# aweisberg/cassandra-accord

Measured on AMD Instinct MI355X. Metric: txn-key conflict pairs resolved/sec (node), higher is better.
Workload: dtype u32/u64 (integer); 1 GPU; config2: KeyDeps batch, 1M txns x 8 keys, zipf(0.99) over 1M keys, p_write 0.5, uncommitted window 10k, per-GPU CommandStore snapshot; key_distribution=zipf, keys_permuted=True, n_txn_per_gpu=1000000, pairs_per_gpu=8000000, dep_edges_per_gpu=35349420, parallelism=keyspace shards x1 (independent CommandStores)

## Files before the change

### cassandra-accord_amd/accord_amd/_lib.py

```python
from __future__ import annotations

import ctypes as C
import os

HERE = os.path.dirname(os.path.abspath(__file__))
LIB_PATH = os.environ.get("ACC_LIB_PATH") or os.path.join(HERE, "libaccord_amd.so")

ACC_OK, ACC_E_ARG, ACC_E_STATE, ACC_E_NOMEM, ACC_E_DEVICE, ACC_E_CAP = 0, -1, -2, -3, -4, -5
ACC_MEM_HOST, ACC_MEM_DEVICE = 0, 1
ACC_OPT_TIMING = 1
ACC_OPT_FORCE_REPLAY = 2
ACC_OPT_NO_WINDOW_TIER = 4
ACC_OPT_TIER_GRID_SHIFT = 16
ACC_OPT_RD_WIDE_SORT = 8
ACC_OPT_PD_SERIAL = 16
ACC_LV_AUTO, ACC_LV_LDS_WALK, ACC_LV_WINDOWED, ACC_LV_WAVES = 0, 1, 2, 3
ACC_STARTED_BEFORE, ACC_STARTED_AFTER, ACC_STARTED_ANY = 0, 1, 2
ACC_DEP_WITH, ACC_DEP_WITHOUT, ACC_DEP_ANY = 0, 1, 2
ACC_STATUS_ANY, ACC_STATUS_IS_PROPOSED, ACC_STATUS_IS_STABLE = 0, 1, 2
ACC_FULL_EXECUTES_AFTER = 1
ACC_LATEST_PROPOSAL, ACC_LATEST_COMMIT = 0, 1
RECOVERY_SCANS = {
    "acceptedOrCommittedStartedBeforeWithoutWitnessing": (ACC_STARTED_BEFORE, ACC_DEP_WITHOUT, ACC_STATUS_IS_PROPOSED, True),
    "stableStartedBeforeAndWitnessed": (ACC_STARTED_BEFORE, ACC_DEP_WITH, ACC_STATUS_IS_STABLE, False),
    "hasAcceptedOrCommittedStartedAfterWithoutWitnessing": (ACC_STARTED_AFTER, ACC_DEP_WITHOUT, ACC_STATUS_IS_PROPOSED, False),
    "hasStableExecutesAfterWithoutWitnessing": (ACC_STARTED_ANY, ACC_DEP_WITHOUT, ACC_STATUS_IS_STABLE, False),
}

u64p = C.POINTER(C.c_uint64)
u32p = C.POINTER(C.c_uint32)
# ... 553 lines not shown
```

### cassandra-accord_amd/accord_amd/deps.py

```python
from __future__ import annotations

import ctypes as C
from dataclasses import dataclass

import numpy as np

from . import _lib as L


class AccordError(RuntimeError):
    code = None


class IllegalArgumentException(AccordError):
    code = L.ACC_E_ARG


class IllegalStateException(AccordError):
    code = L.ACC_E_STATE


class DeviceError(AccordError):
    code = L.ACC_E_DEVICE

# ... 4 lines not shown

_ERRORS = {L.ACC_E_ARG: IllegalArgumentException, L.ACC_E_STATE: IllegalStateException,
           L.ACC_E_DEVICE: DeviceError, L.ACC_E_NOMEM: DeviceError, L.ACC_E_CAP: CapacityError}


def _ptr(a: np.ndarray):
    return C.c_void_p(a.ctypes.data)


class Context:

    LV_TIERS = {"auto": 0, "lds": 1, "windowed": 2, "waves": 3}

    def __init__(self, device: int = 0, timing: bool = False, force_replay: bool = False, *, cfk_hot: int = 0,
                 lv_tier: str = "auto", lv_chunk: int = 0, no_window_tier: bool = False, rd_wide_sort: bool = False,
                 pd_serial: bool = False, cfq_wave_cap: int = 0, wave_grid_max: int = 0, tier_grid_max: int = 0):
        self.timing_enabled = timing
        self.device = device
        self._lib = L.load()
        h = C.c_void_p()
        flags = ((L.ACC_OPT_TIMING if timing else 0) | (L.ACC_OPT_FORCE_REPLAY if force_replay else 0) |
                 (L.ACC_OPT_NO_WINDOW_TIER if no_window_tier else 0) | (L.ACC_OPT_RD_WIDE_SORT if rd_wide_sort else 0) |
                 (L.ACC_OPT_PD_SERIAL if pd_serial else 0))
        if not 0 <= int(tier_grid_max) <= 0xFFFF:
            raise ValueError("tier_grid_max must be within 0..65535")
        flags |= int(tier_grid_max) << L.ACC_OPT_TIER_GRID_SHIFT
        opts = L.Opts(flags, int(wave_grid_max), int(cfk_hot), self.LV_TIERS[lv_tier], int(lv_chunk), int(cfq_wave_cap))
        rc = self._lib.acc_create(device, C.byref(opts), C.byref(h))
        if rc != L.ACC_OK:
            raise _ERRORS.get(rc, AccordError)(f"acc_create failed ({rc})")
        self._h = h
        self._keep = []

    def close(self):
        if getattr(self, "_h", None):
            self._lib.acc_destroy(self._h)
            self._h = None

# ... 1176 lines not shown
```

### cassandra-accord_amd/csrc/api.hip

```cpp
#include "dict.hpp"
#include <exception>
#include <thread>

namespace acc {
void keydeps_batch(acc_ctx *ctx, const acc_batch_in *in, acc_keydeps_view *view);
void keydeps_mixed(acc_ctx *ctx, const acc_range_batch_in *in, acc_keydeps_view *view, SharedDict *shared = nullptr);
void keydeps_merge(acc_ctx *ctx, const acc_merge_in *in, acc_merge_view *view);
void levelise(acc_ctx *ctx, const acc_graph_in *in, uint32_t *level, uint32_t *order, uint32_t *n_levels);
void rangedeps_batch(acc_ctx *ctx, const acc_range_batch_in *in, acc_rangedeps_view *view, const SharedDict *shared = nullptr);
void shard_pack(acc_ctx *ctx, const acc_batch_in *in, acc_frag_streams *out, bool ctx_alloc);
void shard_merge(acc_ctx *ctx, const acc_frag_recv *in, acc_merge_view *view);
void deps_merge(acc_ctx *ctx, const acc_deps_merge_in *in, acc_deps_merge_view *view);
void rmm_invert(acc_ctx *ctx, const acc_rmm_batch *in, acc_csr_view *out);
void rmm_slice(acc_ctx *ctx, const acc_rmm_batch *in, const acc_ranges_in *select, acc_slice_view *out);
void rangedeps_stab(acc_ctx *ctx, const acc_rmm_batch *rd, const acc_stab_in *q, acc_stab_view *out);
void rmm_without(acc_ctx *ctx, const acc_rmm_batch *in, const acc_ts_cols *txn, const acc_txn_sets *set_a,
                 const acc_txn_sets *set_b, acc_without_view *out);
void recovery_deps_reduce(acc_ctx *ctx, const acc_deps_merge_in *cw, const acc_deps_merge_in *anw, acc_recovery_deps_view *view);
void map_reduce_full(acc_ctx *ctx, const acc_batch_in *in, const acc_recovery_in *q, acc_keydeps_view *view);
void map_reduce_full_ranges(acc_ctx *ctx, const acc_range_cmds_in *c, const acc_recovery_ranges_in *q, acc_rangedeps_view *view);
void latest_deps_merge(acc_ctx *ctx, const acc_latest_in *in, acc_latest_view *view);
void deps_from_json(acc_ctx *ctx, const acc_json_in *in, acc_json_deps_view *view);
void deps_to_json(acc_ctx *ctx, const acc_json_out_in *in, acc_json_out *out);
void cfk_update(acc_ctx *ctx, acc_cfk *cfk, const acc_batch_in *in);
// ... 70 lines not shown
{
    if (!ctx) return;
    (void)hipSetDevice(ctx->device);
    if (ctx->stream) (void)hipStreamSynchronize(ctx->stream);
    for (auto &kv : ctx->bufs)
        if (kv.second.ptr) (void)hipFree(kv.second.ptr);
    for (void *p : ctx->graveyard) (void)hipFree(p);
    for (auto &p : ctx->pending) { (void)hipEventDestroy(p.start); (void)hipEventDestroy(p.stop); }
    for (auto e : ctx->event_pool) (void)hipEventDestroy(e);
    for (int i = 0; i < acc_ctx::NAUX; ++i) {
        if (ctx->aux[i]) { (void)hipStreamSynchronize(ctx->aux[i]); (void)hipStreamDestroy(ctx->aux[i]); }
        if (ctx->join_ev[i]) (void)hipEventDestroy(ctx->join_ev[i]);
    }
    if (ctx->fork_ev) (void)hipEventDestroy(ctx->fork_ev);
    if (ctx->lane_ev) (void)hipEventDestroy(ctx->lane_ev);
    if (ctx->pinned) (void)hipHostFree(ctx->pinned);
    if (ctx->stream) (void)hipStreamDestroy(ctx->stream);
    acc_ctx *child = ctx->child;
    delete ctx;
    ctx_destroy(child);
}

}

extern "C" {

const char *acc_last_error(const acc_ctx *ctx) { return ctx ? ctx->last_error.c_str() : "null context"; }

int acc_sync(acc_ctx *ctx)
{
// ... 617 lines not shown
```

### cassandra-accord_amd/csrc/ctx.hpp

```cpp
#pragma once

#include <hip/hip_runtime.h>

#include <algorithm>
#include <cstdint>
#include <cstdio>
#include <cstring>
#include <string>
#include <unordered_map>
#include <vector>

#include "../../include/accord_amd.h"

namespace acc {

struct Error {
    int code;
    std::string msg;
};

[[noreturn]] inline void fail(int code, const std::string &msg) { throw Error{code, msg}; }

constexpr int BLOCK = 256;
constexpr int WAVES = BLOCK / 64;
// ... 20 lines not shown

struct PendingEvent {
    int slot;
    hipEvent_t start, stop;
};

}

struct acc_ctx {
    int device = 0;
    hipStream_t stream = nullptr;
    static constexpr int NAUX = 3;
    hipStream_t aux[NAUX] = {};
    hipEvent_t fork_ev = nullptr, join_ev[NAUX] = {};
    hipEvent_t lane_ev = nullptr;
    bool lane_open = false;
    hipStream_t launch_stream = nullptr;
    struct ScanState {
        size_t cap = 0, dirty[2] = {0, 0};
        int par = 0;
    };
    ScanState scan_st[2];
    int scan_lane() const { return !launch_stream ? 0 : launch_stream == aux[0] ? 1 : -1; }
    struct OsState {
        size_t cap = 0, dirty[2] = {0, 0};
        int par = 0;
    };
    std::unordered_map<std::string, OsState> os_state;
    uint32_t flags = 0;
    acc_opts opts{};
// ... 62 lines not shown
        return static_cast<T *>(b.ptr);
    }

    void swap_buf(const char *name, void *&ptr, size_t &bytes)
    {
        acc::Buf &b = bufs[ns.empty() ? std::string(name) : ns + name];
        std::swap(b.ptr, ptr);
        std::swap(b.bytes, bytes);
    }

    const void *buf_ptr(const char *name) const
    {
        auto it = bufs.find(ns.empty() ? std::string(name) : ns + name);
        return it == bufs.end() ? nullptr : it->second.ptr;
    }

    hipEvent_t take_event()
    {
        if (!event_pool.empty()) {
            hipEvent_t e = event_pool.back();
            event_pool.pop_back();
            return e;
        }
        hipEvent_t e;
        ACC_HIP(hipEventCreate(&e));
        return e;
    }

    int slot(const char *name)
    {
// ... 8 lines not shown
    void resolve_timing()
    {
        for (auto &p : pending) {
            float ms = 0;
            ACC_HIP(hipEventElapsedTime(&ms, p.start, p.stop));
            slots[p.slot].total_ms += ms;
            slots[p.slot].launches += 1;
            event_pool.push_back(p.start);
            event_pool.push_back(p.stop);
        }
        pending.clear();
    }

    hipStream_t cur() const { return launch_stream ? launch_stream : stream; }

    void fork(int k)
    {
        if (!fork_ev) {
            ACC_HIP(hipEventCreateWithFlags(&fork_ev, hipEventDisableTiming));
            ACC_HIP(hipEventCreateWithFlags(&lane_ev, hipEventDisableTiming));
            for (int i = 0; i < NAUX; ++i) {
                ACC_HIP(hipStreamCreateWithFlags(&aux[i], hipStreamNonBlocking));
                ACC_HIP(hipEventCreateWithFlags(&join_ev[i], hipEventDisableTiming));
            }
        }
        ACC_HIP(hipEventRecord(fork_ev, stream));
        for (int i = 0; i < k; ++i) ACC_HIP(hipStreamWaitEvent(aux[i], fork_ev, 0));
    }
    void join(int k)
    {
        for (int i = 0; i < k; ++i) {
            ACC_HIP(hipEventRecord(join_ev[i], aux[i]));
            ACC_HIP(hipStreamWaitEvent(stream, join_ev[i], 0));
        }
        launch_stream = nullptr;
    }

    void lane_fork() { fork(1); lane_open = true; }
    void lane_join() { if (lane_open) { join(1); lane_open = false; } }
    void lane_mark() { ACC_HIP(hipEventRecord(lane_ev, aux[0])); }
    void lane_wait() { ACC_HIP(hipStreamWaitEvent(stream, lane_ev, 0)); }

// ... 112 lines not shown
```

### cassandra-accord_amd/csrc/keydeps.hip

```cpp
#include "keydeps.hpp"

#include <vector>

namespace acc {


struct TxnInfoArgs {
    uint32_t n = 0;
    const uint8_t *status = nullptr;
    const uint64_t *tl = nullptr;
    uint4 *tinfo = nullptr;
    uint32_t *bigflag = nullptr;
};

__device__ __forceinline__ void txn_info_one(uint32_t t, uint32_t n, const uint32_t *rank, const uint8_t *status,
                                             const uint64_t *tl, const uint32_t *key_off, uint4 *tinfo, uint32_t *bigflag)
{
    if (bigflag) bigflag[t] = 0;
    const uint32_t kind = (uint32_t)(tl[t] >> 1) & 7u;
    tinfo[t] = make_uint4(rank[t], rank[n + t], (uint32_t)status[t] | (kind << 3), key_off[t]);
}

__global__ __launch_bounds__(BLOCK) void k_pair_keys(size_t P, const uint64_t *__restrict__ key_code,
                                                     const uint32_t *__restrict__ owner, const uint32_t *__restrict__ key_off,
// ... 1836 lines not shown




constexpr int ST_G = 16;
constexpr int ST_N2 = 128;
constexpr int ST_SLOT = ST_N2;
constexpr uint32_t ST_RAW = 1024;
constexpr int MK_G = 8;

__global__ __launch_bounds__(BLOCK) void k_v3_mark(uint32_t n, const uint32_t *__restrict__ key_off,
                                                   const uint32_t *__restrict__ irec32, const uint4 *__restrict__ rec,
                                                   uint32_t *__restrict__ psz, uint32_t raw_cap,
                                                   uint32_t *__restrict__ bigflag, uint64_t *__restrict__ szA,
                                                   uint64_t *__restrict__ szK, uint64_t *__restrict__ any16,
                                                   uint64_t *__restrict__ eb, uint32_t *__restrict__ runflag)
{
    const uint32_t t = (blockIdx.x * BLOCK + threadIdx.x) / MK_G, sub = threadIdx.x & (MK_G - 1);
    if (t >= n) return;
    const uint32_t j0 = key_off[t], nk = key_off[t + 1] - j0;
    const bool run_rec = bigflag[t] != 0;
    const bool maybe_big = run_rec || nk > 8u;
    uint32_t e = 0, kd = 0, raw = 0;
    for (uint32_t c0 = 0; c0 < nk; c0 += MK_G) {
        if (c0 + sub < nk) {
            const uint32_t w = irec32[IREC_W * (size_t)(j0 + c0 + sub) + 7];
            const uint32_t ej = w & ~REC_INLINE_FLAG;
            e += ej;
            kd += ej != 0;
            if (run_rec && !(w & REC_INLINE_FLAG)) {
                const uint4 *r = rec + 4 * (size_t)(j0 + c0 + sub);
                const uint4 r1 = r[1], r2 = r[2], r3 = r[3];
                raw += r1.z + r1.w + r2.x + r2.y + r2.z + r2.w + r3.y;
            }
            if (maybe_big) psz[j0 + c0 + sub] = ej;
        }
    }
#pragma unroll
    for (int d = 1; d < MK_G; d <<= 1) {
        e += __shfl_xor(e, d, 64);
        kd += __shfl_xor(kd, d, 64);
        raw += __shfl_xor(raw, d, 64);
    }
    const bool big = nk > (uint32_t)ST_G || e > (uint32_t)ST_N2 || (run_rec && raw > raw_cap);
    if (sub == 0) {
        bigflag[t] = big ? 1u : 0u;
        runflag[t] = run_rec && !big ? 1u : 0u;
        szA[t] = (uint64_t)kd + e;
        szK[t] = kd;
        eb[t] = big ? e : 0u;
        if (big && e && nk > 8 && nk <= 16 && !*any16) atomicOr((unsigned long long *)any16, 1ull);
    }
}


__global__ __launch_bounds__(BLOCK) void k_v3_compact(uint32_t n, const uint32_t *__restrict__ bigflag,
                                                      const uint32_t *__restrict__ bpos, uint32_t *__restrict__ blist)
{
    const uint32_t t = blockIdx.x * BLOCK + threadIdx.x;
    if (t < n && bigflag[t]) blist[bpos[t]] = t;
}
__global__ __launch_bounds__(BLOCK) void k_v3_route(uint32_t nbig, const uint32_t *__restrict__ blist,
                                                    const uint32_t *__restrict__ key_off, const uint64_t *__restrict__ eb,
                                                    int big_ok, int win_ok, uint32_t *__restrict__ med_list,
                                                    uint32_t *__restrict__ big_list, uint32_t *__restrict__ fb_list,
                                                    uint32_t *__restrict__ w8_list, uint32_t *__restrict__ w16_list,
                                                    uint64_t *__restrict__ gstat)
{
    const uint32_t i = blockIdx.x * BLOCK + threadIdx.x;
    bool med = false, bg = false, fb = false, w8 = false, w16 = false;
    uint32_t t = 0;
    uint64_t E = 0;
    if (i < nbig) {
        t = blist[i];
        E = eb[t];
// ... 76 lines not shown
            b.u_cnt[t] = 0;
        }
    }
}

struct V3Stream {
    V2View v;
    const uint32_t *key_off, *bigflag, *txn_of_rank;
    const uint32_t *list;
    const uint4 *rec, *irec;
    const uint64_t *arena_off, *kd_off;
    uint64_t *u_cnt_out;
    int32_t *arena;
    uint32_t *key_idx, *dep_scr;
    uint64_t *err;
    uint32_t n, ntiles;
};

template <int G>
__device__ __forceinline__ uint32_t group_inclusive(uint32_t x, uint32_t sub)
{
#pragma unroll
    for (uint32_t d = 1; d < (uint32_t)G; d <<= 1) {
        const uint32_t u = __shfl_up(x, d, 64);
        if (sub >= d) x += u;
    }
    return x;
}

template <class T>
// ... 35 lines not shown
            }
        }
    }
#pragma unroll
    for (int r = 0; r < R; ++r) buf[r * G + sub] = v[r];
}

#ifdef ACC_PHASE_PROF
__device__ unsigned long long *g_st_prof;
__device__ unsigned long long *g_sr_prof;
#define ST_PH(i) ph[i] = clock64()
#else
#define ST_PH(i) ((void)0)
#endif

#ifndef ACC_ST_WAVES
#define ACC_ST_WAVES 24
#endif
template <class EntT, int NT, int G, int N2, bool LIST, bool RUNS>
__global__ __launch_bounds__(NT, ACC_ST_WAVES * 64 / NT) void k_v3_stream(V3Stream s)
{
    constexpr int TT = NT / G;
    constexpr uint32_t KB = G <= 8 ? 3 : 4;
    static_assert(G <= 16, "entries keep the key index in 4 bits");
#ifdef ACC_PHASE_PROF
    uint64_t ph[8];
#endif
    ST_PH(0);
    __shared__ EntT ent[TT][N2];
    __shared__ uint32_t kc[TT][G];
    __shared__ uint32_t kbase[TT][G];
    __shared__ uint16_t stA[TT][G + N2];
    const uint32_t tid = threadIdx.x, lane = lane_id(), sub = lane & (G - 1), grp = tid / G, g0 = lane & (64 - G);
    const uint64_t gmask = ((1ull << G) - 1) << g0;
    const uint64_t lt = lane == 0 ? 0ull : (~0ull >> (64 - lane));
    const uint32_t tile = blockIdx.x * (NT / 64) + (tid >> 6);
    const uint32_t slot = tile * (64 / G) + lane / G;
    const bool valid = slot < s.n;
    const uint32_t t = LIST ? (valid ? s.list[slot] : 0u) : slot;
    TxnCtx c{};
    bool big = false;
    uint64_t aoff = 0, koff = 0;
    if (valid) {
        c.t = t;
        c.j0 = s.key_off[t]; c.j1 = s.key_off[t + 1];
        const uint32_t bf = s.bigflag[t];
        const uint4 ti = s.v.tinfo[t];
        aoff = s.arena_off[t]; koff = s.kd_off[t];
        c.nk = c.j1 - c.j0;
        big = bf != 0;
        c.trank = ti.x;
        c.bq = ti.y != c.trank;
        c.wk = witnesses(ti.z >> 3);
    }
// ... 440 lines not shown
    cb.tm = stage_in(ctx, "in_tm", in->txn_id.msb, n, in->mem);
    cb.tl = stage_in(ctx, "in_tl", in->txn_id.lsb, n, in->mem);
    cb.tn = stage_in(ctx, "in_tn", in->txn_id.node, n, in->mem);
    cb.em = stage_in(ctx, "in_em", in->execute_at.msb, n, in->mem);
    cb.el = stage_in(ctx, "in_el", in->execute_at.lsb, n, in->mem);
    cb.en = stage_in(ctx, "in_en", in->execute_at.node, n, in->mem);
    cb.status = stage_in(ctx, "in_status", in->status, n, in->mem);
    cb.key_code = stage_in(ctx, "in_key_code", in->key_code, P, in->mem);

    cb.g = ctx->get<uint64_t>("g", PREP_G_WORDS);
    cb.owner = ctx->get<uint32_t>("owner", P);
    prep_batch(ctx, n, P, cb.tm, cb.tl, cb.tn, cb.em, cb.el, cb.en, cb.status, cb.key_off, cb.key_code, cb.owner, cb.g, cb.dict);
    const bool overlap = pair_plan(cb) && cb.dict.fast_ok && cb.pp.rk.bits + cb.dict.rbits + 1 <= 64;
    ctx->stat("keydeps.build_overlap", overlap ? 1 : 0);
    ctx->stat("keydeps.bc_sort_passes", 0);
    if (overlap) ctx->lane_fork();
    else build_dictionary(ctx, n, cb.tm, cb.tl, cb.tn, cb.em, cb.el, cb.en, cb.g, cb.dict, true);

    cb.tinfo = ctx->get<uint4>("tinfo", n);
    cb.bigflag = ctx->get<uint32_t>("v3_bigflag", n);
    const PairSort ps = sort_pairs(ctx, cb, overlap);
    if (overlap) {
        ctx->launch_stream = ctx->aux[0];
        build_dictionary(ctx, n, cb.tm, cb.tl, cb.tn, cb.em, cb.el, cb.en, cb.g, cb.dict, true);
        ctx->lane_mark();
        bc_from_txns(ctx, cb);
        ctx->launch_stream = nullptr;
    }
    cb.perm = ps.ps.vals;
    if (!ps.flags_done)
// ... 124 lines not shown
    }

    V2View vv{};
    vv.perm = cb.perm; vv.pair_pos = cb.pair_pos; vv.seg_incl = cb.seg_incl; vv.seg_start = cb.seg_start;
    vv.s_rank = cb.s_rank; vv.s_exec = cb.s_exec; vv.s_info = cb.s_info; vv.rdir = cols.rdir; vv.tinfo = cb.tinfo;
    vv.list_rank = cols.list_rank; vv.bases = cb.bases; vv.bc_rank = cols.bc_rank; vv.bc_exec = cols.bc_exec; vv.bc_pm = bc_pm64;
    vv.bc_kind = cols.bc_kind; vv.bcs_exec = bcs_exec; vv.bcs_lastw = bcs_lw64;
    if (P >= 0x80000000ull) fail(ACC_E_CAP, "n_pairs must be < 2^31 (count-pass record format)");
    RecOut ro;
    ro.rec = ctx->get<uint4>("v2_rec", 4 * P);
    ro.irec = ctx->get<uint4>("v2_irec", 2 * P);
    uint4 *rec = ro.rec;
    vv.irec32 = reinterpret_cast<const uint32_t *>(ro.irec);
    vv.rec = ro.rec;

    uint32_t *bpos = ctx->get<uint32_t>("v3_bpos", n);
    uint64_t *blk_e = ctx->get<uint64_t>("v3_blk_e", gP);
    uint32_t *psz = ctx->get<uint32_t>("v3_psz", P);
#ifdef ACC_PHASE_PROF
    const size_t ct_rows = (size_t)gP * WAVES;
    unsigned long long *ct_buf = prof_arm(ctx, "v2_ct_prof", HIP_SYMBOL(g_ct_prof), 8 * ct_rows, st);
#endif
    launch(ctx, "v2_count", k_v2_count, dim3(gP), dim3(BLOCK), 0, P, vv, (const uint32_t *)owner, ro, bigflag, blk_e);
#ifdef ACC_PHASE_PROF
    {
        const std::vector<unsigned long long> h = prof_read(ct_buf, 8 * ct_rows, st);
        double sum[8] = {}, mx[3] = {};
        size_t w = 0;
        for (size_t r = 0; r < ct_rows; ++r) {
            if (!(h[8 * r + 7] >> 32)) continue;
            ++w;
// ... 1 lines not shown
            sum[7] += (double)(h[8 * r + 7] & 0xFFFFFFFFu);
            for (int i = 0; i < 3; ++i) mx[i] = std::max(mx[i], (double)h[8 * r + i]);
        }
        const double d = w ? (double)w : 1.0;
        fprintf(stderr, "[ct_phase] waves=%zu avg cycles: query %.0f r3count %.0f inline+write %.0f | max %.0f %.0f %.0f | "
                "per pair: bumped %.4f seg-with-bc %.4f posM-search %.4f r3-candidates %.3f run-records %.4f\n",
                w, sum[0] / d, sum[1] / d, sum[2] / d, mx[0], mx[1], mx[2], sum[3] / P, sum[4] / P, sum[5] / P, sum[6] / P,
                sum[7] / P);
    }
#endif
    const uint32_t raw_cap = ST_RAW;
    uint64_t *kd_off = ctx->get<uint64_t>("kd_off", (size_t)n + 1);
    uint64_t *arena_off = ctx->get<uint64_t>("arena_off", (size_t)n + 1);
    uint64_t *szA = ctx->get<uint64_t>("v3_szA", n), *szK = ctx->get<uint64_t>("v3_szK", n);
    uint64_t *eb = ctx->get<uint64_t>("v3_eb", n), *dB = ctx->get<uint64_t>("v3_dB", (size_t)n + 1);
    uint32_t *runflag = ctx->get<uint32_t>("v3_runflag", n);
    launch(ctx, "v3_mark", k_v3_mark, dim3(grid_for((size_t)n * MK_G, BLOCK)), dim3(BLOCK), 0, n, key_off,
           (const uint32_t *)ro.irec, (const uint4 *)rec, psz, raw_cap, bigflag, szA, szK, tot + 2, eb, runflag);
    uint64_t *blk_pre = ctx->get<uint64_t>("v3_blk_pre", gP);
    {
        const uint64_t *si[4] = { szA, szK, blk_e, eb };
        uint64_t *so[4] = { arena_off, kd_off, blk_pre, dB }, *stot[4] = { arena_off + n, kd_off + n, tot, dB + n };
        const size_t sn[4] = { n, n, gP, n };
        scan_multi<uint64_t, OpAdd<uint64_t>>(ctx, 4, si, so, sn, true, stot);
    }
    scan<uint32_t, OpAdd<uint32_t>>(ctx, bigflag, bpos, n, true, reinterpret_cast<uint32_t *>(tot + 1));
    uint32_t *blist = ctx->get<uint32_t>("v3_blist", n);
    launch(ctx, "v3_compact", k_v3_compact, dim3(grid_for(n, BLOCK)), dim3(BLOCK), 0, n, (const uint32_t *)bigflag,
           (const uint32_t *)bpos, blist);
    uint32_t *rpos = ctx->get<uint32_t>("v3_rpos", n), *rlist = ctx->get<uint32_t>("v3_rlist", n);
    scan<uint32_t, OpAdd<uint32_t>>(ctx, runflag, rpos, n, true, reinterpret_cast<uint32_t *>(tot + 3));
    launch(ctx, "v3_compact", k_v3_compact, dim3(grid_for(n, BLOCK)), dim3(BLOCK), 0, n, (const uint32_t *)runflag,
           (const uint32_t *)rpos, rlist);
    ACC_HIP(hipMemcpyAsync(ctx->pinned, tot, 4 * sizeof(uint64_t), hipMemcpyDeviceToHost, st));
    ctx->sync();
    const uint64_t E = ctx->pinned[0];
    const uint32_t nbig = (uint32_t)ctx->pinned[1];
    const bool any16 = ctx->pinned[2] != 0;
    const uint32_t nrun = (uint32_t)ctx->pinned[3];
    if (E >= 0xFFFFFFFFull) fail(ACC_E_CAP, "more than 2^32-1 dependency entries in one batch");
    uint64_t *u_off = ctx->get<uint64_t>("u_off", (size_t)n + 1);
    uint64_t *u_cnt = ctx->get<uint64_t>("u_cnt", n);
    uint64_t *vdep_off = nullptr;
    uint32_t *dep_scr = nullptr;
    uint64_t nfb = 0, efb = 0, nmed = 0, nbig2 = 0;
    ctx->stat("keydeps.huge_txns", 0);
    V2Out wo{};
    bool win_ok = false;
#ifdef ACC_PHASE_PROF
    unsigned long long *win_buf = nullptr, *sr_buf = nullptr;
    size_t sr_rows = 0;
#endif
    uint64_t *vcnt = nullptr;
    uint32_t *med_list = nullptr, *big_list = nullptr, *fb_list = nullptr;
    const unsigned tgm = (ctx->flags >> ACC_OPT_TIER_GRID_SHIFT) ? (ctx->flags >> ACC_OPT_TIER_GRID_SHIFT) : ~0u;
    auto tier_grid = [&](unsigned work, unsigned dflt) { return dim3(std::max(1u, std::min(std::min(work, dflt), tgm))); };
    auto sort_tiers = [&](bool with_med) {
        if (with_med)
            launch(ctx, "v2_write_med", k_v2_write_big<MED_CAP, BLOCK>, tier_grid(nbig, 2048), dim3(BLOCK), 0,
                   (const uint32_t *)med_list, vv, (const uint64_t *)vcnt, wo);
        launch(ctx, "v2_write_big", k_v2_write_big<BIG_E, 512>, tier_grid(nbig, 1024), dim3(512), 0,
               (const uint32_t *)big_list, vv, (const uint64_t *)vcnt, wo);
        launch(ctx, "v2_write_huge", k_v2_write_big<HUGE_E, 1024>, tier_grid(nbig, 64), dim3(1024), 0,
               (const uint32_t *)wo.huge_list, vv, (const uint64_t *)vcnt, wo);
    };
    uint32_t *dep_st = ctx->get<uint32_t>("v3_dep_stream", (size_t)n * ST_SLOT);
    int32_t *const arena = ctx->get<int32_t>("arena", P + E);
    uint32_t *const key_idx = ctx->get<uint32_t>("key_idx", P);
    uint32_t *const dep_txn = ctx->get<uint32_t>("dep_txn", std::max<uint64_t>(E, 1));
    auto finish = [&]() {
        scan<uint64_t, OpAdd<uint64_t>>(ctx, u_cnt, u_off, n, true, u_off + n);
        const uint32_t *tmap = nullptr, *ne_cnt = nullptr;
        const uint64_t *uo = u_off;
        if (cb.opts.sparse) {
            uint32_t *flag = ctx->get<uint32_t>("v3_ne_flag", n), *pos = ctx->get<uint32_t>("v3_ne_pos", n);
            uint32_t *cnt = ctx->get<uint32_t>("v3_ne_cnt", 1), *ne_t = ctx->get<uint32_t>("v3_ne_t", n);
            uint64_t *ne_uoff = ctx->get<uint64_t>("v3_ne_uoff", (size_t)n + 1);
            launch(ctx, "v3_neflag", k_v3_neflag, dim3(grid_for(n, BLOCK)), dim3(BLOCK), 0, n, (const uint64_t *)u_cnt, flag);
            scan<uint32_t, OpAdd<uint32_t>>(ctx, flag, pos, n, true, cnt);
            launch(ctx, "v3_nelist", k_v3_nelist, dim3(grid_for(n, BLOCK)), dim3(BLOCK), 0, n, (const uint32_t *)flag,
                   (const uint32_t *)pos, (const uint32_t *)cnt, (const uint64_t *)u_off, ne_t, ne_uoff);
            tmap = ne_t; ne_cnt = cnt; uo = ne_uoff;
        }
        launch(ctx, "v3_ucompact", k_v3_ucompact, dim3((unsigned)((E + UC_CHUNK - 1) / UC_CHUNK) + 1), dim3(BLOCK), 0, n,
               uo, (const uint64_t *)arena_off, (const uint64_t *)kd_off, (const uint32_t *)bigflag, key_off,
               (const uint64_t *)vdep_off, (const uint32_t *)dep_st, (const uint32_t *)dep_scr,
               tmap, ne_cnt, dep_txn, (const uint64_t *)u_off, gstat + GSTAT_N);
        ACC_HIP(hipMemcpyAsync(ctx->pinned, gstat, (GSTAT_N + 6) * sizeof(uint64_t), hipMemcpyDeviceToHost, st));
        ctx->sync();
    };
    if (nbig) {
        const unsigned gB = (nbig + WAVES - 1) / WAVES;
        vdep_off = ctx->get<uint64_t>("dep_off", P + 1);
        vcnt = ctx->get<uint64_t>("cnt", P);
        uint32_t *vcnz = ctx->get<uint32_t>("cnz", P + 1);
        dep_scr = ctx->get<uint32_t>("v2_dep_scratch", std::max<uint64_t>(E, 1));
        med_list = ctx->get<uint32_t>("v2_med_list", nbig);
        big_list = ctx->get<uint32_t>("v2_big_list", nbig);
        fb_list = ctx->get<uint32_t>("v2_fb_list", nbig);
        V3Big bg;
        bg.blist = blist; bg.key_off = key_off; bg.psz = psz; bg.dB = dB; bg.arena_off = arena_off; bg.kd_off = kd_off;
        bg.vdep_off = vdep_off; bg.vcnt = vcnt; bg.vcnz = vcnz; bg.u_cnt = u_cnt; bg.arena = arena; bg.key_idx = key_idx;
        const bool big_ok = rbits + 6 <= 31;
        win_ok = big_ok && !(ctx->flags & ACC_OPT_NO_WINDOW_TIER);
        launch(ctx, "v3_route", k_v3_route, dim3(grid_for(nbig, BLOCK)), dim3(BLOCK), 0, nbig, (const uint32_t *)blist,
               key_off, (const uint64_t *)eb, (int)big_ok, (int)win_ok, med_list, big_list, fb_list,
               ctx->get<uint32_t>("v2_w8_list", nbig), ctx->get<uint32_t>("v2_w16_list", nbig), gstat);
        launch(ctx, "v3_bigfill", k_v3_bigfill, dim3(gB), dim3(BLOCK), 0, nbig, bg);
        wo.key_off = key_off; wo.dep_off = vdep_off; wo.arena_off = arena_off; wo.cnz = vcnz; wo.txn_of_rank = txn_of_rank;
        wo.arena = arena; wo.dep_scratch = dep_scr; wo.u_cnt = u_cnt; wo.gstat = gstat;
        wo.rec = rec; wo.irec32 = vv.irec32; wo.med_list = med_list; wo.big_list = big_list; wo.fb_list = fb_list;
        wo.huge_list = ctx->get<uint32_t>("v2_huge_list", nbig);
        ctx->fork(nrun ? 2 : 1);
        ctx->launch_stream = ctx->aux[0];
        if (win_ok) {
#ifdef ACC_PHASE_PROF
            win_buf = prof_arm(ctx, "v2_win_prof", HIP_SYMBOL(g_win_prof), 10, ctx->aux[0]);
#endif
            launch(ctx, "v2_write_win", k_v2_write_win<8>, tier_grid(nbig, 2048), dim3(BLOCK), 0,
                   (const uint32_t *)ctx->get<uint32_t>("v2_w8_list", nbig), (const uint64_t *)(gstat + 7), vv,
                   (const uint64_t *)vcnt, wo);
            if (any16)
                launch(ctx, "v2_write_win16", k_v2_write_win<16>, tier_grid(nbig, 256), dim3(BLOCK), 0,
                       (const uint32_t *)ctx->get<uint32_t>("v2_w16_list", nbig), (const uint64_t *)(gstat + 8), vv,
                       (const uint64_t *)vcnt, wo);
        } else if (big_ok) {
            sort_tiers(true);
        } else {
            launch(ctx, "v2_write_medium", k_v2_write_medium, tier_grid(gB, 2048), dim3(BLOCK), 0,
                   (const uint64_t *)gstat, (const uint32_t *)med_list, vv, (const uint64_t *)vcnt, wo);
        }
        ctx->launch_stream = nullptr;
    }
    {
        constexpr int st_nt = 256;
        const uint32_t tt = (uint32_t)st_nt / ST_G;
        const uint32_t nblocks = (n + tt - 1) / tt;
        const uint32_t ntiles = nblocks * (uint32_t)(st_nt / 64);
        V3Stream sp;
        sp.v = vv; sp.err = gstat + 5;
        sp.key_off = key_off; sp.bigflag = bigflag; sp.list = nullptr; sp.txn_of_rank = txn_of_rank;
        sp.rec = rec; sp.irec = ro.irec;
        sp.arena_off = arena_off; sp.kd_off = kd_off; sp.u_cnt_out = u_cnt; sp.arena = arena; sp.key_idx = key_idx;
        sp.dep_scr = dep_st; sp.n = n; sp.ntiles = ntiles;
#ifdef ACC_PHASE_PROF
        const size_t prof_rows = (size_t)ntiles;
        unsigned long long *prof_buf = prof_arm(ctx, "v3_prof", HIP_SYMBOL(g_st_prof), 8 * prof_rows, st);
#endif
        if (nrun) {
            if (!nbig) ctx->fork(2);
            V3Stream sr = sp;
            sr.list = rlist; sr.n = nrun;
            const uint32_t rblocks = (nrun + tt - 1) / tt;
            ctx->launch_stream = ctx->aux[1];
#ifdef ACC_PHASE_PROF
            sr_rows = (size_t)rblocks * (st_nt / 64);
            sr_buf = prof_arm(ctx, "v3_sr_prof", HIP_SYMBOL(g_sr_prof), 8 * sr_rows, ctx->aux[1]);
#endif
            if (rbits <= 28) launch(ctx, "v3_stream_runs", k_v3_stream<uint32_t, st_nt, ST_G, ST_N2, true, true>, dim3(rblocks), dim3(st_nt), 0, sr);
            else launch(ctx, "v3_stream_runs", k_v3_stream<uint64_t, st_nt, ST_G, ST_N2, true, true>, dim3(rblocks), dim3(st_nt), 0, sr);
            ctx->launch_stream = nullptr;
        }
        if (rbits <= 28) launch(ctx, "v3_stream", k_v3_stream<uint32_t, st_nt, ST_G, ST_N2, false, false>, dim3(nblocks), dim3(st_nt), 0, sp);
        else launch(ctx, "v3_stream", k_v3_stream<uint64_t, st_nt, ST_G, ST_N2, false, false>, dim3(nblocks), dim3(st_nt), 0, sp);
#ifdef ACC_PHASE_PROF
        {
            const std::vector<unsigned long long> h = prof_read(prof_buf, 8 * prof_rows, st);
            double sum[6] = {}, mx[6] = {};
            size_t w = 0;
            for (size_t r = 0; r < prof_rows; ++r) {
                if (!h[8 * r + 7]) continue;
                ++w;
                for (int i = 0; i < 6; ++i) { sum[i] += (double)h[8 * r + i]; mx[i] = std::max(mx[i], (double)h[8 * r + i]); }
            }
            const double d = w ? (double)w : 1.0;
            fprintf(stderr, "[st_phase] waves=%zu avg cycles: setup %.0f records %.0f gather %.0f sort %.0f emit-lds %.0f lookback+copy %.0f | max: %.0f %.0f %.0f %.0f %.0f %.0f\n",
                    w, sum[0] / d, sum[1] / d, sum[2] / d, sum[3] / d, sum[4] / d, sum[5] / d, mx[0], mx[1], mx[2], mx[3], mx[4], mx[5]);
        }
#endif
    }
    if (nbig || nrun) ctx->join(nrun ? 2 : 1);
#ifdef ACC_PHASE_PROF
    if (nbig && win_ok) {
        const std::vector<unsigned long long> h = prof_read(win_buf, 10, st);
        const double nt = h[6] ? (double)h[6] : 1.0;
        fprintf(stderr, "[win_phase] txns=%llu avg cycles per txn (thread 0 of each block): lowend %.0f gather %.0f "
                "union %.0f sort|prefix|below %.0f span-writes %.0f list-wait %.0f | avg E %.1f span words %.1f below %.1f\n",
                h[6], h[0] / nt, h[1] / nt, h[2] / nt, h[3] / nt, h[4] / nt, h[9] / nt, h[7] / nt,
                (double)(h[8] >> 32) / nt, (double)(h[8] & 0xFFFFFFFFull) / nt);
    }
#endif
#ifdef ACC_PHASE_PROF
    if (sr_buf) {
        const std::vector<unsigned long long> h = prof_read(sr_buf, 8 * sr_rows, st);
        double sum[6] = {};
        size_t w = 0;
// ... 83 lines not shown
```

### cassandra-accord_amd/csrc/prims.hpp

```cpp
#pragma once

#include "ctx.hpp"

#include <algorithm>
#include <vector>

namespace acc {


__device__ __forceinline__ uint32_t lane_id() { return threadIdx.x & 63u; }

template <class T>
__device__ __forceinline__ T shfl_up(T v, unsigned d)
{
    if constexpr (sizeof(T) == 8) {
        uint64_t u = (uint64_t)v;
        uint32_t lo = __shfl_up((uint32_t)u, d, 64), hi = __shfl_up((uint32_t)(u >> 32), d, 64);
        return (T)(((uint64_t)hi << 32) | lo);
    } else {
        return (T)__shfl_up((uint32_t)v, d, 64);
    }
}

template <class T>
// ... 161 lines not shown
    }
}


constexpr uint64_t SCAN_AGG = 1ull << 62, SCAN_INC = 2ull << 62, SCAN_VAL = (1ull << 62) - 1;

__device__ __forceinline__ void scan_status_store(uint64_t *p, uint64_t w)
{
    __hip_atomic_store(p, w, __ATOMIC_RELAXED, __HIP_MEMORY_SCOPE_AGENT);
}
__device__ __forceinline__ uint64_t scan_status_load(const uint64_t *p)
{
    return __hip_atomic_load(p, __ATOMIC_RELAXED, __HIP_MEMORY_SCOPE_AGENT);
}

constexpr int SCAN_MAXA = 4;
template <class T>
struct ScanArgs {
    const T *in[SCAN_MAXA];
    T *out[SCAN_MAXA];
    T *total[SCAN_MAXA];
    uint64_t n[SCAN_MAXA];
    uint32_t cum[SCAN_MAXA + 1];
    int k;
};

template <class T, class Op, int ITEMS>
__global__ __launch_bounds__(BLOCK) void k_scan_1p(ScanArgs<T> a, int exclusive, uint32_t *__restrict__ ticket,
                                                 uint64_t *__restrict__ status, uint64_t *__restrict__ other, uint32_t other_n)
{
    constexpr int TILE = BLOCK * ITEMS;
// ... 678 lines not shown
```

### include/accord_amd.h

```cpp
#ifndef ACCORD_AMD_H
#define ACCORD_AMD_H

#include <stdint.h>
#include <stddef.h>

#ifdef __cplusplus
extern "C" {
#endif

typedef struct acc_rlist {
    const uint64_t *start;
    const uint64_t *end;
    uint32_t n;
    uint32_t reserved;
} acc_rlist;

#define ACC_OK          0
#define ACC_E_ARG      (-1)
#define ACC_E_STATE    (-2)
#define ACC_E_NOMEM    (-3)
#define ACC_E_DEVICE   (-4)
#define ACC_E_CAP      (-5)

#define ACC_ST_TRANSITIVELY_KNOWN   0
// ... 10 lines not shown
#define ACC_KIND_EPHEMERAL_READ       2
#define ACC_KIND_SYNC_POINT           3
#define ACC_KIND_EXCLUSIVE_SYNC_POINT 4
#define ACC_KIND_LOCAL_ONLY           5

#define ACC_MEM_HOST   0
#define ACC_MEM_DEVICE 1

#define ACC_OPT_TIMING 0x1u
#define ACC_OPT_FORCE_REPLAY 0x2u
#define ACC_OPT_NO_WINDOW_TIER 0x4u
#define ACC_OPT_RD_WIDE_SORT 0x8u
#define ACC_OPT_TIER_GRID_SHIFT 16
#define ACC_OPT_TIER_GRID(n) ((uint32_t)(n) << ACC_OPT_TIER_GRID_SHIFT)
#define ACC_OPT_PD_SERIAL 0x10u

#define ACC_LV_AUTO     0u
#define ACC_LV_LDS_WALK 1u
#define ACC_LV_WINDOWED 2u
#define ACC_LV_WAVES    3u

typedef struct acc_ctx acc_ctx;

typedef struct acc_opts {
    uint32_t flags;
    uint32_t wave_grid_max;
    uint32_t cfk_hot;
    uint32_t lv_tier;
    uint32_t lv_chunk;
    uint32_t cfq_wave_cap;
// ... 673 lines not shown
```

Measured before the change: 3.714 billion txn-key pairs/s.

## Stream-ahead lean pass during host readback and merge list compaction scans

Packs the big and run flags into one 64-bit word so both compaction lists come out of one fused multi-scan and one list kernel, replacing two separate scans and compactions. It also launches the first 1/8 of the lean stream pass speculatively into the previously allocated arena before the host reads back the entry totals. The kernel checks on the device whether the arena is large enough and exits if not, and the host syncs and redoes the work when capacity is insufficient. Side streams now fork at the readback event, which adds ordering complexity and the risk of wasted speculative work.

```diff
diff --git a/cassandra-accord_amd/accord_amd/_lib.py b/cassandra-accord_amd/accord_amd/_lib.py
--- a/cassandra-accord_amd/accord_amd/_lib.py
+++ b/cassandra-accord_amd/accord_amd/_lib.py
@@ -14,6 +14,7 @@
 ACC_OPT_TIER_GRID_SHIFT = 16
 ACC_OPT_RD_WIDE_SORT = 8
 ACC_OPT_PD_SERIAL = 16
+ACC_OPT_KD_NO_STREAM_AHEAD = 32
 ACC_LV_AUTO, ACC_LV_LDS_WALK, ACC_LV_WINDOWED, ACC_LV_WAVES = 0, 1, 2, 3
 ACC_STARTED_BEFORE, ACC_STARTED_AFTER, ACC_STARTED_ANY = 0, 1, 2
 ACC_DEP_WITH, ACC_DEP_WITHOUT, ACC_DEP_ANY = 0, 1, 2
diff --git a/cassandra-accord_amd/accord_amd/deps.py b/cassandra-accord_amd/accord_amd/deps.py
--- a/cassandra-accord_amd/accord_amd/deps.py
+++ b/cassandra-accord_amd/accord_amd/deps.py
@@ -42,14 +42,16 @@
 
     def __init__(self, device: int = 0, timing: bool = False, force_replay: bool = False, *, cfk_hot: int = 0,
                  lv_tier: str = "auto", lv_chunk: int = 0, no_window_tier: bool = False, rd_wide_sort: bool = False,
-                 pd_serial: bool = False, cfq_wave_cap: int = 0, wave_grid_max: int = 0, tier_grid_max: int = 0):
+                 pd_serial: bool = False, cfq_wave_cap: int = 0, wave_grid_max: int = 0, tier_grid_max: int = 0,
+                 no_stream_ahead: bool = False):
         self.timing_enabled = timing
         self.device = device
         self._lib = L.load()
         h = C.c_void_p()
         flags = ((L.ACC_OPT_TIMING if timing else 0) | (L.ACC_OPT_FORCE_REPLAY if force_replay else 0) |
                  (L.ACC_OPT_NO_WINDOW_TIER if no_window_tier else 0) | (L.ACC_OPT_RD_WIDE_SORT if rd_wide_sort else 0) |
-                 (L.ACC_OPT_PD_SERIAL if pd_serial else 0))
+                 (L.ACC_OPT_PD_SERIAL if pd_serial else 0) |
+                 (L.ACC_OPT_KD_NO_STREAM_AHEAD if no_stream_ahead else 0))
         if not 0 <= int(tier_grid_max) <= 0xFFFF:
             raise ValueError("tier_grid_max must be within 0..65535")
         flags |= int(tier_grid_max) << L.ACC_OPT_TIER_GRID_SHIFT
diff --git a/cassandra-accord_amd/csrc/api.hip b/cassandra-accord_amd/csrc/api.hip
--- a/cassandra-accord_amd/csrc/api.hip
+++ b/cassandra-accord_amd/csrc/api.hip
@@ -108,6 +108,7 @@
     }
     if (ctx->fork_ev) (void)hipEventDestroy(ctx->fork_ev);
     if (ctx->lane_ev) (void)hipEventDestroy(ctx->lane_ev);
+    if (ctx->read_ev) (void)hipEventDestroy(ctx->read_ev);
     if (ctx->pinned) (void)hipHostFree(ctx->pinned);
     if (ctx->stream) (void)hipStreamDestroy(ctx->stream);
     acc_ctx *child = ctx->child;
diff --git a/cassandra-accord_amd/csrc/ctx.hpp b/cassandra-accord_amd/csrc/ctx.hpp
--- a/cassandra-accord_amd/csrc/ctx.hpp
+++ b/cassandra-accord_amd/csrc/ctx.hpp
@@ -58,6 +58,7 @@
     hipStream_t aux[NAUX] = {};
     hipEvent_t fork_ev = nullptr, join_ev[NAUX] = {};
     hipEvent_t lane_ev = nullptr;
+    hipEvent_t read_ev = nullptr;
     bool lane_open = false;
     hipStream_t launch_stream = nullptr;
     struct ScanState {
@@ -150,6 +151,11 @@
         auto it = bufs.find(ns.empty() ? std::string(name) : ns + name);
         return it == bufs.end() ? nullptr : it->second.ptr;
     }
+    size_t buf_cap(const char *name) const
+    {
+        auto it = bufs.find(ns.empty() ? std::string(name) : ns + name);
+        return it == bufs.end() || !it->second.ptr ? 0 : it->second.bytes;
+    }
 
     hipEvent_t take_event()
     {
@@ -188,18 +194,32 @@
 
     hipStream_t cur() const { return launch_stream ? launch_stream : stream; }
 
+    void need_aux()
+    {
+        if (fork_ev) return;
+        ACC_HIP(hipEventCreateWithFlags(&fork_ev, hipEventDisableTiming));
+        ACC_HIP(hipEventCreateWithFlags(&lane_ev, hipEventDisableTiming));
+        ACC_HIP(hipEventCreateWithFlags(&read_ev, hipEventDisableTiming));
+        for (int i = 0; i < NAUX; ++i) {
+            ACC_HIP(hipStreamCreateWithFlags(&aux[i], hipStreamNonBlocking));
+            ACC_HIP(hipEventCreateWithFlags(&join_ev[i], hipEventDisableTiming));
+        }
+    }
     void fork(int k)
     {
-        if (!fork_ev) {
-            ACC_HIP(hipEventCreateWithFlags(&fork_ev, hipEventDisableTiming));
-            ACC_HIP(hipEventCreateWithFlags(&lane_ev, hipEventDisableTiming));
-            for (int i = 0; i < NAUX; ++i) {
-                ACC_HIP(hipStreamCreateWithFlags(&aux[i], hipStreamNonBlocking));
-                ACC_HIP(hipEventCreateWithFlags(&join_ev[i], hipEventDisableTiming));
-            }
-        }
+        need_aux();
         ACC_HIP(hipEventRecord(fork_ev, stream));
         for (int i = 0; i < k; ++i) ACC_HIP(hipStreamWaitEvent(aux[i], fork_ev, 0));
+    }
+    void read_mark()
+    {
+        need_aux();
+        ACC_HIP(hipEventRecord(read_ev, stream));
+    }
+    void read_wait() { ACC_HIP(hipEventSynchronize(read_ev)); }
+    void fork_at_read(int k)
+    {
+        for (int i = 0; i < k; ++i) ACC_HIP(hipStreamWaitEvent(aux[i], read_ev, 0));
     }
     void join(int k)
     {
diff --git a/cassandra-accord_amd/csrc/keydeps.hip b/cassandra-accord_amd/csrc/keydeps.hip
--- a/cassandra-accord_amd/csrc/keydeps.hip
+++ b/cassandra-accord_amd/csrc/keydeps.hip
@@ -1874,7 +1874,7 @@
                                                    uint32_t *__restrict__ psz, uint32_t raw_cap,
                                                    uint32_t *__restrict__ bigflag, uint64_t *__restrict__ szA,
                                                    uint64_t *__restrict__ szK, uint64_t *__restrict__ any16,
-                                                   uint64_t *__restrict__ eb, uint32_t *__restrict__ runflag)
+                                                   uint64_t *__restrict__ eb, uint64_t *__restrict__ flagw)
 {
     const uint32_t t = (blockIdx.x * BLOCK + threadIdx.x) / MK_G, sub = threadIdx.x & (MK_G - 1);
     if (t >= n) return;
@@ -1905,7 +1905,7 @@
     const bool big = nk > (uint32_t)ST_G || e > (uint32_t)ST_N2 || (run_rec && raw > raw_cap);
     if (sub == 0) {
         bigflag[t] = big ? 1u : 0u;
-        runflag[t] = run_rec && !big ? 1u : 0u;
+        flagw[t] = (big ? 1ull : 0ull) | (run_rec && !big ? 1ull << 32 : 0ull);
         szA[t] = (uint64_t)kd + e;
         szK[t] = kd;
         eb[t] = big ? e : 0u;
@@ -1914,11 +1914,17 @@
 }
 
 
-__global__ __launch_bounds__(BLOCK) void k_v3_compact(uint32_t n, const uint32_t *__restrict__ bigflag,
-                                                      const uint32_t *__restrict__ bpos, uint32_t *__restrict__ blist)
+__global__ __launch_bounds__(BLOCK) void k_v3_lists(uint32_t n, const uint64_t *__restrict__ flagw,
+                                                    const uint64_t *__restrict__ fpos, uint32_t *__restrict__ blist,
+                                                    uint32_t *__restrict__ rlist)
 {
     const uint32_t t = blockIdx.x * BLOCK + threadIdx.x;
-    if (t < n && bigflag[t]) blist[bpos[t]] = t;
+    if (t >= n) return;
+    const uint64_t f = flagw[t];
+    if (!f) return;
+    const uint64_t p = fpos[t];
+    if (f & 1u) blist[(uint32_t)p] = t;
+    else rlist[(uint32_t)(p >> 32)] = t;
 }
 __global__ __launch_bounds__(BLOCK) void k_v3_route(uint32_t nbig, const uint32_t *__restrict__ blist,
                                                     const uint32_t *__restrict__ key_off, const uint64_t *__restrict__ eb,
@@ -2025,6 +2031,9 @@
     int32_t *arena;
     uint32_t *key_idx, *dep_scr;
     uint64_t *err;
+    const uint64_t *e_dev;
+    uint64_t pairs, arena_cap;
+    uint32_t t0;
     uint32_t n, ntiles;
 };
 
@@ -2090,6 +2099,9 @@
 #define ST_PH(i) ((void)0)
 #endif
 
+#ifndef ACC_AHEAD_DIV
+#define ACC_AHEAD_DIV 8
+#endif
 #ifndef ACC_ST_WAVES
 #define ACC_ST_WAVES 24
 #endif
@@ -2103,6 +2115,7 @@
     uint64_t ph[8];
 #endif
     ST_PH(0);
+    if (s.e_dev && s.pairs + *s.e_dev > s.arena_cap) return;
     __shared__ EntT ent[TT][N2];
     __shared__ uint32_t kc[TT][G];
     __shared__ uint32_t kbase[TT][G];
@@ -2113,7 +2126,7 @@
     const uint32_t tile = blockIdx.x * (NT / 64) + (tid >> 6);
     const uint32_t slot = tile * (64 / G) + lane / G;
     const bool valid = slot < s.n;
-    const uint32_t t = LIST ? (valid ? s.list[slot] : 0u) : slot;
+    const uint32_t t = LIST ? (valid ? s.list[slot] : 0u) : s.t0 + slot;
     TxnCtx c{};
     bool big = false;
     uint64_t aoff = 0, koff = 0;
@@ -2584,6 +2597,8 @@
     const bool overlap = pair_plan(cb) && cb.dict.fast_ok && cb.pp.rk.bits + cb.dict.rbits + 1 <= 64;
     ctx->stat("keydeps.build_overlap", overlap ? 1 : 0);
     ctx->stat("keydeps.bc_sort_passes", 0);
+    ctx->stat("keydeps.stream_ahead", 0);
+    ctx->stat("keydeps.stream_ahead_redo", 0);
     if (overlap) ctx->lane_fork();
     else build_dictionary(ctx, n, cb.tm, cb.tl, cb.tn, cb.em, cb.el, cb.en, cb.g, cb.dict, true);
 
@@ -2738,7 +2753,6 @@
     vv.irec32 = reinterpret_cast<const uint32_t *>(ro.irec);
     vv.rec = ro.rec;
 
-    uint32_t *bpos = ctx->get<uint32_t>("v3_bpos", n);
     uint64_t *blk_e = ctx->get<uint64_t>("v3_blk_e", gP);
     uint32_t *psz = ctx->get<uint32_t>("v3_psz", P);
 #ifdef ACC_PHASE_PROF
@@ -2770,33 +2784,69 @@
     uint64_t *arena_off = ctx->get<uint64_t>("arena_off", (size_t)n + 1);
     uint64_t *szA = ctx->get<uint64_t>("v3_szA", n), *szK = ctx->get<uint64_t>("v3_szK", n);
     uint64_t *eb = ctx->get<uint64_t>("v3_eb", n), *dB = ctx->get<uint64_t>("v3_dB", (size_t)n + 1);
-    uint32_t *runflag = ctx->get<uint32_t>("v3_runflag", n);
+    if (n >= (1u << 30)) fail(ACC_E_CAP, "n_txn must be < 2^30 (list flags scanned as one word)");
+    uint64_t *flagw = ctx->get<uint64_t>("v3_flagw", n), *fpos = ctx->get<uint64_t>("v3_fpos", n);
     launch(ctx, "v3_mark", k_v3_mark, dim3(grid_for((size_t)n * MK_G, BLOCK)), dim3(BLOCK), 0, n, key_off,
-           (const uint32_t *)ro.irec, (const uint4 *)rec, psz, raw_cap, bigflag, szA, szK, tot + 2, eb, runflag);
+           (const uint32_t *)ro.irec, (const uint4 *)rec, psz, raw_cap, bigflag, szA, szK, tot + 2, eb, flagw);
     uint64_t *blk_pre = ctx->get<uint64_t>("v3_blk_pre", gP);
     {
-        const uint64_t *si[4] = { szA, szK, blk_e, eb };
-        uint64_t *so[4] = { arena_off, kd_off, blk_pre, dB }, *stot[4] = { arena_off + n, kd_off + n, tot, dB + n };
-        const size_t sn[4] = { n, n, gP, n };
-        scan_multi<uint64_t, OpAdd<uint64_t>>(ctx, 4, si, so, sn, true, stot);
-    }
-    scan<uint32_t, OpAdd<uint32_t>>(ctx, bigflag, bpos, n, true, reinterpret_cast<uint32_t *>(tot + 1));
-    uint32_t *blist = ctx->get<uint32_t>("v3_blist", n);
-    launch(ctx, "v3_compact", k_v3_compact, dim3(grid_for(n, BLOCK)), dim3(BLOCK), 0, n, (const uint32_t *)bigflag,
-           (const uint32_t *)bpos, blist);
-    uint32_t *rpos = ctx->get<uint32_t>("v3_rpos", n), *rlist = ctx->get<uint32_t>("v3_rlist", n);
-    scan<uint32_t, OpAdd<uint32_t>>(ctx, runflag, rpos, n, true, reinterpret_cast<uint32_t *>(tot + 3));
-    launch(ctx, "v3_compact", k_v3_compact, dim3(grid_for(n, BLOCK)), dim3(BLOCK), 0, n, (const uint32_t *)runflag,
-           (const uint32_t *)rpos, rlist);
-    ACC_HIP(hipMemcpyAsync(ctx->pinned, tot, 4 * sizeof(uint64_t), hipMemcpyDeviceToHost, st));
-    ctx->sync();
-    const uint64_t E = ctx->pinned[0];
-    const uint32_t nbig = (uint32_t)ctx->pinned[1];
-    const bool any16 = ctx->pinned[2] != 0;
-    const uint32_t nrun = (uint32_t)ctx->pinned[3];
-    if (E >= 0xFFFFFFFFull) fail(ACC_E_CAP, "more than 2^32-1 dependency entries in one batch");
+        const uint64_t *si[5] = { szA, szK, blk_e, eb, flagw };
+        uint64_t *so[5] = { arena_off, kd_off, blk_pre, dB, fpos };
+        uint64_t *stot[5] = { arena_off + n, kd_off + n, tot, dB + n, tot + 1 };
+        const size_t sn[5] = { n, n, gP, n, n };
+        scan_multi<uint64_t, OpAdd<uint64_t>>(ctx, 5, si, so, sn, true, stot);
+    }
+    uint32_t *blist = ctx->get<uint32_t>("v3_blist", n), *rlist = ctx->get<uint32_t>("v3_rlist", n);
+    launch(ctx, "v3_lists", k_v3_lists, dim3(grid_for(n, BLOCK)), dim3(BLOCK), 0, n, (const uint64_t *)flagw,
+           (const uint64_t *)fpos, blist, rlist);
+    ACC_HIP(hipMemcpyAsync(ctx->pinned, tot, 3 * sizeof(uint64_t), hipMemcpyDeviceToHost, st));
+    ctx->read_mark();
+    const uint64_t arena_cap = ctx->buf_cap("arena") / sizeof(int32_t);
+    bool ahead = arena_cap != 0 && !(ctx->flags & ACC_OPT_KD_NO_STREAM_AHEAD);
+#ifdef ACC_PHASE_PROF
+    ahead = false;
+#endif
     uint64_t *u_off = ctx->get<uint64_t>("u_off", (size_t)n + 1);
     uint64_t *u_cnt = ctx->get<uint64_t>("u_cnt", n);
+    uint32_t *dep_st = ctx->get<uint32_t>("v3_dep_stream", (size_t)n * ST_SLOT);
+    uint32_t *const key_idx = ctx->get<uint32_t>("key_idx", P);
+    constexpr int st_nt = 256;
+    const uint32_t tt = (uint32_t)st_nt / ST_G;
+    const uint32_t nblocks = (n + tt - 1) / tt;
+    const uint32_t ntiles = nblocks * (uint32_t)(st_nt / 64);
+    V3Stream sp;
+    sp.v = vv; sp.err = gstat + 5;
+    sp.key_off = key_off; sp.bigflag = bigflag; sp.list = nullptr; sp.txn_of_rank = txn_of_rank;
+    sp.rec = rec; sp.irec = ro.irec;
+    sp.arena_off = arena_off; sp.kd_off = kd_off; sp.u_cnt_out = u_cnt; sp.arena = nullptr; sp.key_idx = key_idx;
+    sp.dep_scr = dep_st; sp.t0 = 0; sp.n = n; sp.ntiles = ntiles;
+    sp.e_dev = nullptr; sp.pairs = P; sp.arena_cap = arena_cap;
+    auto lean_pass = [&](uint32_t t0, uint32_t cnt) {
+        V3Stream a = sp;
+        a.t0 = t0; a.n = cnt;
+        const uint32_t nb = (cnt + tt - 1) / tt;
+        if (rbits <= 28) launch(ctx, "v3_stream", k_v3_stream<uint32_t, st_nt, ST_G, ST_N2, false, false>, dim3(nb), dim3(st_nt), 0, a);
+        else launch(ctx, "v3_stream", k_v3_stream<uint64_t, st_nt, ST_G, ST_N2, false, false>, dim3(nb), dim3(st_nt), 0, a);
+    };
+    const uint32_t n_ahead = ahead ? n / ACC_AHEAD_DIV / tt * tt : 0u;
+    if (ahead) {
+        sp.arena = static_cast<int32_t *>(const_cast<void *>(ctx->buf_ptr("arena")));
+        sp.e_dev = tot;
+        lean_pass(0, n_ahead);
+    }
+    ctx->read_wait();
+    const uint64_t E = ctx->pinned[0];
+    const uint32_t nbig = (uint32_t)(ctx->pinned[1] & 0xFFFFFFFFu);
+    const uint32_t nrun = (uint32_t)(ctx->pinned[1] >> 32);
+    const bool any16 = ctx->pinned[2] != 0;
+    if (E >= 0xFFFFFFFFull) fail(ACC_E_CAP, "more than 2^32-1 dependency entries in one batch");
+    const bool redo = ahead && P + E > arena_cap;
+    if (redo) {
+        ctx->sync();
+        ahead = false;
+    }
+    ctx->stat("keydeps.stream_ahead", ahead ? 1 : 0);
+    ctx->stat("keydeps.stream_ahead_redo", redo ? 1 : 0);
     uint64_t *vdep_off = nullptr;
     uint32_t *dep_scr = nullptr;
     uint64_t nfb = 0, efb = 0, nmed = 0, nbig2 = 0;
@@ -2820,9 +2870,8 @@
         launch(ctx, "v2_write_huge", k_v2_write_big<HUGE_E, 1024>, tier_grid(nbig, 64), dim3(1024), 0,
                (const uint32_t *)wo.huge_list, vv, (const uint64_t *)vcnt, wo);
     };
-    uint32_t *dep_st = ctx->get<uint32_t>("v3_dep_stream", (size_t)n * ST_SLOT);
     int32_t *const arena = ctx->get<int32_t>("arena", P + E);
-    uint32_t *const key_idx = ctx->get<uint32_t>("key_idx", P);
+    sp.arena = arena; sp.e_dev = nullptr;
     uint32_t *const dep_txn = ctx->get<uint32_t>("dep_txn", std::max<uint64_t>(E, 1));
     auto finish = [&]() {
         scan<uint64_t, OpAdd<uint64_t>>(ctx, u_cnt, u_off, n, true, u_off + n);
@@ -2845,6 +2894,8 @@
         ACC_HIP(hipMemcpyAsync(ctx->pinned, gstat, (GSTAT_N + 6) * sizeof(uint64_t), hipMemcpyDeviceToHost, st));
         ctx->sync();
     };
+    const int nside = nrun ? 2 : nbig ? 1 : 0;
+    if (ahead) ctx->fork_at_read(nside);
     if (nbig) {
         const unsigned gB = (nbig + WAVES - 1) / WAVES;
         vdep_off = ctx->get<uint64_t>("dep_off", P + 1);
@@ -2859,15 +2910,21 @@
         bg.vdep_off = vdep_off; bg.vcnt = vcnt; bg.vcnz = vcnz; bg.u_cnt = u_cnt; bg.arena = arena; bg.key_idx = key_idx;
         const bool big_ok = rbits + 6 <= 31;
         win_ok = big_ok && !(ctx->flags & ACC_OPT_NO_WINDOW_TIER);
+        if (ahead) ctx->launch_stream = ctx->aux[0];
         launch(ctx, "v3_route", k_v3_route, dim3(grid_for(nbig, BLOCK)), dim3(BLOCK), 0, nbig, (const uint32_t *)blist,
                key_off, (const uint64_t *)eb, (int)big_ok, (int)win_ok, med_list, big_list, fb_list,
                ctx->get<uint32_t>("v2_w8_list", nbig), ctx->get<uint32_t>("v2_w16_list", nbig), gstat);
         launch(ctx, "v3_bigfill", k_v3_bigfill, dim3(gB), dim3(BLOCK), 0, nbig, bg);
+        if (ahead) {
+            ctx->lane_mark();
+            ctx->lane_wait();
+            if (nrun) ACC_HIP(hipStreamWaitEvent(ctx->aux[1], ctx->lane_ev, 0));
+        }
         wo.key_off = key_off; wo.dep_off = vdep_off; wo.arena_off = arena_off; wo.cnz = vcnz; wo.txn_of_rank = txn_of_rank;
         wo.arena = arena; wo.dep_scratch = dep_scr; wo.u_cnt = u_cnt; wo.gstat = gstat;
         wo.rec = rec; wo.irec32 = vv.irec32; wo.med_list = med_list; wo.big_list = big_list; wo.fb_list = fb_list;
         wo.huge_list = ctx->get<uint32_t>("v2_huge_list", nbig);
-        ctx->fork(nrun ? 2 : 1);
+        if (!ahead) ctx->fork(nside);
         ctx->launch_stream = ctx->aux[0];
         if (win_ok) {
 #ifdef ACC_PHASE_PROF
@@ -2889,22 +2946,12 @@
         ctx->launch_stream = nullptr;
     }
     {
-        constexpr int st_nt = 256;
-        const uint32_t tt = (uint32_t)st_nt / ST_G;
-        const uint32_t nblocks = (n + tt - 1) / tt;
-        const uint32_t ntiles = nblocks * (uint32_t)(st_nt / 64);
-        V3Stream sp;
-        sp.v = vv; sp.err = gstat + 5;
-        sp.key_off = key_off; sp.bigflag = bigflag; sp.list = nullptr; sp.txn_of_rank = txn_of_rank;
-        sp.rec = rec; sp.irec = ro.irec;
-        sp.arena_off = arena_off; sp.kd_off = kd_off; sp.u_cnt_out = u_cnt; sp.arena = arena; sp.key_idx = key_idx;
-        sp.dep_scr = dep_st; sp.n = n; sp.ntiles = ntiles;
 #ifdef ACC_PHASE_PROF
         const size_t prof_rows = (size_t)ntiles;
         unsigned long long *prof_buf = prof_arm(ctx, "v3_prof", HIP_SYMBOL(g_st_prof), 8 * prof_rows, st);
 #endif
         if (nrun) {
-            if (!nbig) ctx->fork(2);
+            if (!nbig && !ahead) ctx->fork(2);
             V3Stream sr = sp;
             sr.list = rlist; sr.n = nrun;
             const uint32_t rblocks = (nrun + tt - 1) / tt;
@@ -2917,8 +2964,7 @@
             else launch(ctx, "v3_stream_runs", k_v3_stream<uint64_t, st_nt, ST_G, ST_N2, true, true>, dim3(rblocks), dim3(st_nt), 0, sr);
             ctx->launch_stream = nullptr;
         }
-        if (rbits <= 28) launch(ctx, "v3_stream", k_v3_stream<uint32_t, st_nt, ST_G, ST_N2, false, false>, dim3(nblocks), dim3(st_nt), 0, sp);
-        else launch(ctx, "v3_stream", k_v3_stream<uint64_t, st_nt, ST_G, ST_N2, false, false>, dim3(nblocks), dim3(st_nt), 0, sp);
+        lean_pass(ahead ? n_ahead : 0u, ahead ? n - n_ahead : n);
 #ifdef ACC_PHASE_PROF
         {
             const std::vector<unsigned long long> h = prof_read(prof_buf, 8 * prof_rows, st);
@@ -2935,7 +2981,7 @@
         }
 #endif
     }
-    if (nbig || nrun) ctx->join(nrun ? 2 : 1);
+    if (nside) ctx->join(nside);
 #ifdef ACC_PHASE_PROF
     if (nbig && win_ok) {
         const std::vector<unsigned long long> h = prof_read(win_buf, 10, st);
diff --git a/cassandra-accord_amd/csrc/prims.hpp b/cassandra-accord_amd/csrc/prims.hpp
--- a/cassandra-accord_amd/csrc/prims.hpp
+++ b/cassandra-accord_amd/csrc/prims.hpp
@@ -199,7 +199,7 @@
     return __hip_atomic_load(p, __ATOMIC_RELAXED, __HIP_MEMORY_SCOPE_AGENT);
 }
 
-constexpr int SCAN_MAXA = 4;
+constexpr int SCAN_MAXA = 5;
 template <class T>
 struct ScanArgs {
     const T *in[SCAN_MAXA];
diff --git a/include/accord_amd.h b/include/accord_amd.h
--- a/include/accord_amd.h
+++ b/include/accord_amd.h
@@ -48,6 +48,7 @@
 #define ACC_OPT_TIER_GRID_SHIFT 16
 #define ACC_OPT_TIER_GRID(n) ((uint32_t)(n) << ACC_OPT_TIER_GRID_SHIFT)
 #define ACC_OPT_PD_SERIAL 0x10u
+#define ACC_OPT_KD_NO_STREAM_AHEAD 0x20u
 
 #define ACC_LV_AUTO     0u
 #define ACC_LV_LDS_WALK 1u
```

Result: faster. 3.964 billion txn-key pairs/s, median of 6 (+6.7%).
